# ZhonghuaYi/EI-Nexus_official

Hardware: AMD Instinct MI355X
Metric: event-image pairs/s (extract+match, 346x260, 1024 kpts) (higher is better)
Workload: dtype f32; 1 GPU; B32 346x260 5-bin event voxel + gray image, VGG(event)+SuperPoint(image) extractors, MNN matcher, k=1024; global_batch=32, event_bins=5, parallelism=dp1 (pairs sharded, metric all-reduce only), log_assignment=False, dense_outputs=False, same_scene_pairs=False, weights=seeded synthetic, descriptor-head bias calibrated (per-channel mean removed)

## Files before the change

### ei-nexus_official_amd/_lib.py

```python
import ctypes
import os

_HERE = os.path.dirname(os.path.abspath(__file__))
LIB_PATH = os.environ.get("EINX_LIB") or os.path.join(_HERE, "libeinx_hip.so")

c_void_p, c_int, c_float, c_size_t, c_char_p = ctypes.c_void_p, ctypes.c_int, ctypes.c_float, ctypes.c_size_t, ctypes.c_char_p


class ConvDesc(ctypes.Structure):
    _fields_ = [("w_native", c_void_p), ("bias", c_void_p), ("scale", c_void_p), ("shift", c_void_p),
                ("cin", ctypes.c_int32), ("cout", ctypes.c_int32), ("ks", ctypes.c_int32), ("relu", ctypes.c_int32),
                ("pool", ctypes.c_int32)]


class DetectParams(ctypes.Structure):
    _fields_ = [("B", ctypes.c_int32), ("Hp", ctypes.c_int32), ("Wp", ctypes.c_int32), ("H", ctypes.c_int32),
                ("W", ctypes.c_int32), ("h0", ctypes.c_int32), ("w0", ctypes.c_int32), ("radius", ctypes.c_int32),
                ("top_k", ctypes.c_int32), ("det_thr", c_float), ("ordering_xy", ctypes.c_int32), ("cap", ctypes.c_int32),
                ("nms_iters", ctypes.c_int32)]


class ExtractorDesc(ctypes.Structure):
    _fields_ = [("struct_size", c_size_t), ("cell", ctypes.c_int32), ("n_backbone", ctypes.c_int32), ("n_det", ctypes.c_int32), ("n_desc", ctypes.c_int32),
                ("backbone", ctypes.POINTER(ConvDesc)), ("det_head", ctypes.POINTER(ConvDesc)), ("desc_head", ctypes.POINTER(ConvDesc)),
# ... 11 lines not shown
              "sparse_desc")
    _fields_ = [(n, c_void_p) for n in _names] + [("cap", ctypes.c_int32), ("score_crop", c_void_p)]


class WeightWatch(ctypes.Structure):
    _fields_ = [("struct_size", c_size_t), ("n", ctypes.c_int32), ("table", c_void_p), ("ref", c_void_p), ("scratch", c_void_p), ("stale", c_void_p)]


class MetricParams(ctypes.Structure):
    _fields_ = [(n, ctypes.c_int32) for n in ("B", "cap0", "cap1", "D", "cols", "H0", "W0", "H1", "W1", "kp_yx", "n_mma", "n_vdd")] + \
               [("mma_thr", c_float * 4), ("vdd_thr", c_float * 4), ("rep_nan_if_empty", ctypes.c_int32)]


class PoseParams(ctypes.Structure):
    _fields_ = [("struct_size", c_size_t)] + [(n, ctypes.c_int32) for n in ("B", "cap", "cols", "kp_yx", "k_f64", "max_iters")] + \
               [("thresh", ctypes.c_double), ("conf", ctypes.c_double), ("seed", ctypes.c_uint64)]


class HomographyParams(ctypes.Structure):
    _fields_ = [("struct_size", c_size_t)] + [(n, ctypes.c_int32) for n in ("B", "cap", "cols", "kp_yx", "max_iters", "n_thr")] + \
               [("thresh", ctypes.c_double), ("conf", ctypes.c_double), ("he_thr", c_float * 4), ("seed", ctypes.c_uint64)]


class GtMatchesParams(ctypes.Structure):
    _fields_ = [("struct_size", c_size_t)] + [(n, ctypes.c_int32) for n in ("B", "cap0", "cap1", "cols0", "cols1", "kp_yx", "H0", "W0", "H1", "W1",
                                                                            "homography")] + [("pos_sq", c_float), ("neg_sq", c_float)]


class EventArrays(ctypes.Structure):
    _fields_ = [("x", c_void_p), ("y", c_void_p), ("t", c_void_p), ("p", c_void_p), ("x_type", ctypes.c_int32), ("y_type", ctypes.c_int32),
                ("t_type", ctypes.c_int32), ("p_type", ctypes.c_int32), ("n", ctypes.c_int64)]


class LgLayer(ctypes.Structure):
    _names = ("Wqkv", "bqkv", "Wo", "bo", "sf0_w", "sf0_b", "sln_g", "sln_b", "sf3_w", "sf3_b",
              "Wqk", "bqk", "Wv", "bv", "Wco", "bco", "cf0_w", "cf0_b", "cln_g", "cln_b", "cf3_w", "cf3_b", "Wqk_v", "bqk_v")
    _fields_ = [(n, c_void_p) for n in _names]


class LgWeights(ctypes.Structure):
    _fields_ = [("struct_size", c_size_t), ("layer_size", c_size_t), ("in_w", c_void_p), ("in_b", c_void_p), ("Wr", c_void_p), ("proj_w", c_void_p), ("proj_b", c_void_p),
                ("match_w", c_void_p), ("match_b", c_void_p), ("n_layers", ctypes.c_int32), ("heads", ctypes.c_int32),
                ("d", ctypes.c_int32), ("input_dim", ctypes.c_int32), ("filter_threshold", c_float),
                ("layers", ctypes.POINTER(LgLayer))]


class LgHead(ctypes.Structure):
    _fields_ = [(n, c_void_p) for n in ("proj_w", "proj_b", "match_w", "match_b", "token_w", "token_b")]


SIGNATURES = {
    "einx_version": (c_char_p, []),
    "einx_abi_version": (c_int, []),
    "einx_build_flags": (c_char_p, []),
    "einx_params_hash": (c_int, [c_void_p, c_int, c_void_p, c_void_p, c_void_p, c_void_p]),
    "einx_last_error": (c_char_p, []),
    "einx_math_eval": (c_int, [c_int, c_void_p, ctypes.c_longlong, c_void_p, c_void_p]),
    "einx_fork_stream_of": (c_void_p, [c_void_p]),
    "einx_fork_stream_prepare_beside": (c_int, [c_void_p, ctypes.POINTER(c_void_p), c_int]),
    "einx_stream_overlap_us": (c_int, [c_void_p, c_void_p, c_int, ctypes.POINTER(ctypes.c_float)]),
    "einx_device_count": (c_int, []),
    "einx_profile_enable": (c_int, [c_int]),
    "einx_profile_report": (c_int, [c_char_p, c_size_t]),
    "einx_extractor_create": (c_void_p, [ctypes.POINTER(ExtractorDesc)]),
    "einx_extractor_destroy": (None, [c_void_p]),
    "einx_fork_stream_prepare": (c_int, [c_void_p]),
    "einx_fork_stream_release": (c_int, [c_void_p]),
    "einx_fork_stream_count": (c_int, []),
    "einx_side_stream": (c_void_p, [c_void_p, c_int, ctypes.POINTER(c_void_p), c_int]),
    "einx_extract_shapes": (c_int, [c_void_p, c_int, c_int, ctypes.POINTER(ExtractShapes)]),
    "einx_extract_ws_bytes": (c_size_t, [c_void_p, c_int, c_int, c_int, c_int, c_int]),
    "einx_extract": (c_int, [c_void_p, c_void_p, c_void_p, c_int, c_int, c_int, c_int, c_void_p, c_size_t, ctypes.POINTER(ExtractOut), c_void_p]),
    "einx_extract_watch": (c_int, [c_void_p, c_void_p, c_void_p, c_int, c_int, c_int, c_int, c_void_p, c_size_t, ctypes.POINTER(ExtractOut),
                           ctypes.POINTER(WeightWatch), c_void_p]),
    "einx_conv_last_kernel": (c_char_p, []),
    "einx_conv_plan": (c_char_p, [c_int] * 11),
    "einx_conv_weight_elems": (c_size_t, [c_int, c_int, c_int]),
    "einx_conv_repack": (c_int, [c_void_p, c_int, c_int, c_int, c_void_p, c_void_p]),
    "einx_bn_fold": (c_int, [c_void_p, c_void_p, c_void_p, c_void_p, c_float, c_int, c_void_p, c_void_p, c_void_p]),
    "einx_conv_block": (c_int, [c_void_p, c_int, c_int, c_int, c_int, c_int, c_int, c_int, ctypes.POINTER(ConvDesc), c_void_p, c_void_p]),
    "einx_conv_first_two_fused_ok": (c_int, [ctypes.POINTER(ConvDesc), ctypes.POINTER(ConvDesc), c_int, c_int, c_int]),
    "einx_conv_first_two_fused": (c_int, [c_void_p, c_int, c_int, c_int, c_int, c_int, c_int, c_int, ctypes.POINTER(ConvDesc), ctypes.POINTER(ConvDesc),
                                  c_void_p, c_void_p]),
    "einx_div_inplace": (c_int, [c_void_p, c_size_t, c_float, c_void_p]),
    "einx_image_prepare": (c_int, [c_void_p, c_int, c_int, c_int, c_int, ctypes.c_longlong, ctypes.c_longlong, ctypes.c_longlong, ctypes.c_longlong,
                           c_float, c_void_p, c_void_p]),
    "einx_score_map": (c_int, [c_void_p, c_int, c_int, c_int, c_int, c_void_p, c_int, c_int, c_int, c_int, c_int, c_int, c_void_p,
                               c_void_p, c_void_p]),
    "einx_remove_border": (c_int, [c_void_p, c_int, c_int, c_int, c_int, c_void_p]),
    "einx_detect_ws_bytes": (c_size_t, [ctypes.POINTER(DetectParams)]),
    "einx_detect": (c_int, [c_void_p, ctypes.POINTER(DetectParams), c_void_p, c_void_p, c_void_p, c_void_p, c_void_p, c_void_p,
                            c_void_p, c_void_p]),
    "einx_desc_sample": (c_int, [c_void_p, c_int, c_int, c_int, c_int, c_int, c_int, c_int, c_int, c_void_p, c_void_p, c_int, c_float,
                                 c_void_p, c_void_p]),
    "einx_normalize_map": (c_int, [c_void_p, c_int, c_int, c_int, c_float, c_void_p, c_void_p, c_void_p]),
    "einx_upsample_ws_bytes": (c_size_t, [c_int, c_int, c_int]),
    "einx_upsample_normalize": (c_int, [c_void_p, c_int, c_int, c_int, c_int, c_int, c_int, c_int, c_int, c_int, c_int, c_float,
                                        c_void_p, c_void_p, c_size_t, c_void_p]),
    "einx_mnn_ws_bytes": (c_size_t, [c_int, c_int, c_int]),
    "einx_mnn": (c_int, [c_void_p, c_void_p, c_int, c_void_p, c_void_p, c_int, c_int, c_int, c_void_p, c_void_p, c_void_p, c_void_p,
                         c_void_p, c_void_p, c_void_p]),
    "einx_mnn_gather": (c_int, [c_void_p, c_void_p, c_int, c_void_p, c_void_p, c_int, c_int, c_int, c_void_p, c_void_p, c_void_p, c_void_p,
                                c_void_p, c_void_p, c_void_p, c_void_p, c_int, c_void_p, c_void_p, c_void_p, c_void_p]),
    "einx_mnn_thresh": (c_int, [c_void_p, c_void_p, c_int, c_void_p, c_void_p, c_int, c_int, c_int, c_int, c_float, c_int, c_float, c_void_p,
                                c_void_p, c_void_p, c_void_p, c_void_p, c_void_p, c_void_p]),
    "einx_gather_matches": (c_int, [c_void_p, c_void_p, c_void_p, c_void_p, c_int, c_int, c_int, c_int, c_void_p, c_void_p, c_void_p,
                                    c_void_p]),
    "einx_events_ws_bytes": (c_size_t, [c_int, c_int, c_int]),
    "einx_voxel_ws_bytes": (c_size_t, [c_int, c_int, c_int, c_int, ctypes.c_int64]),
    "einx_voxel_grid": (c_int, [c_void_p, c_void_p, c_void_p, c_void_p, c_void_p, c_int, c_int, c_int, c_int, c_int, c_void_p, c_void_p,
                                c_size_t, c_void_p]),
    "einx_events_mask": (c_int, [c_void_p, c_void_p, c_void_p, c_int, c_int, c_int, c_void_p, c_void_p, c_void_p]),
    "einx_time_surface_ws_bytes": (c_size_t, [c_int, c_int, c_int, c_int, ctypes.c_int64]),
    "einx_event_stack_ws_bytes": (c_size_t, [c_int, c_int, c_int, c_int, ctypes.c_int64]),
    "einx_distance_map_ws_bytes": (c_size_t, [c_int, c_int, c_int, c_int, ctypes.c_int64]),
    "einx_time_surface": (c_int, [c_void_p, c_void_p, c_void_p, c_void_p, c_void_p, c_int, c_int, c_int, c_int, c_void_p, c_void_p, c_size_t,
                                  c_void_p]),
    "einx_event_stack": (c_int, [c_void_p, c_void_p, c_void_p, c_void_p, c_void_p, c_int, c_int, c_int, c_int, c_void_p, c_void_p, c_size_t,
                                 c_void_p]),
    "einx_distance_map": (c_int, [c_void_p, c_void_p, c_void_p, c_void_p, c_void_p, c_int, c_int, c_int, c_int, c_void_p, c_void_p, c_size_t,
                                  c_void_p]),
    "einx_distance_map_plan": (c_char_p, [c_int, c_int]),
    "einx_events_windows_ws_bytes": (c_size_t, [c_int, c_int, c_int]),
    "einx_voxel_windows_ws_bytes": (c_size_t, [c_int, c_int, c_int, c_int, ctypes.c_int64]),
    "einx_voxel_grid_windows": (c_int, [c_void_p, c_void_p, c_void_p, c_void_p, ctypes.c_int64, c_void_p, c_void_p, c_int, c_int, c_int, c_int, c_int,
                                        c_void_p, c_void_p, c_size_t, c_void_p]),
    "einx_events_mask_windows": (c_int, [c_void_p, c_void_p, ctypes.c_int64, c_void_p, c_void_p, c_int, c_int, c_int, c_void_p, c_size_t, c_void_p,
                                         c_void_p]),
    "einx_events_pack": (c_int, [ctypes.POINTER(EventArrays), c_int, c_void_p, c_void_p, c_void_p, c_void_p, c_void_p, c_int]),
    "einx_metrics_ws_bytes": (c_size_t, [ctypes.POINTER(MetricParams)]),
    "einx_pair_metrics": (c_int, [ctypes.POINTER(MetricParams)] + [c_void_p] * 13),
    "einx_relative_pose_ws_bytes": (c_size_t, [ctypes.POINTER(PoseParams)]),
    "einx_relative_pose": (c_int, [ctypes.POINTER(PoseParams)] + [c_void_p] * 13),
    "einx_essential_5pt": (c_int, [c_void_p, c_void_p, c_int, c_void_p, c_void_p, c_void_p]),
    "einx_homography_ws_bytes": (c_size_t, [ctypes.POINTER(HomographyParams)]),
    "einx_homography": (c_int, [ctypes.POINTER(HomographyParams)] + [c_void_p] * 11),
    "einx_homography_dlt": (c_int, [c_void_p, c_void_p, c_int, c_int, c_void_p, c_void_p, c_void_p]),
    "einx_gt_matches_ws_bytes": (c_size_t, [ctypes.POINTER(GtMatchesParams)]),
    "einx_gt_project": (c_int, [ctypes.POINTER(GtMatchesParams)] + [c_void_p] * 23),
    "einx_gt_warp": (c_int, [ctypes.POINTER(GtMatchesParams)] + [c_void_p] * 8),
    "einx_gt_label": (c_int, [ctypes.POINTER(GtMatchesParams)] + [c_void_p] * 17),
    "einx_gt_matches": (c_int, [ctypes.POINTER(GtMatchesParams)] + [c_void_p] * 30),
    "einx_match_pr": (c_int, [c_void_p, c_void_p, c_void_p, c_void_p, c_int, c_int, c_void_p, c_void_p]),
    "einx_desc_loss_ws_bytes": (c_size_t, [c_int] * 11),
    "einx_desc_loss": (c_int, [c_void_p, c_float, c_void_p, c_float] + [c_int] * 11 + [c_void_p, c_int, c_int, c_void_p, c_void_p, c_size_t, c_void_p]),
    "einx_map_loss_ws_bytes": (c_size_t, [c_int, c_int]),
    "einx_map_loss": (c_int, [c_void_p, c_void_p, c_int, c_int, c_int, c_void_p, c_int, c_int, c_int, c_void_p, c_void_p, c_size_t, c_void_p]),
    "einx_logits_loss": (c_int, [c_void_p, c_void_p] + [c_int] * 9 + [c_void_p, c_int, c_void_p, c_void_p, c_size_t, c_void_p]),
    "einx_linear": (c_int, [c_void_p, c_int, c_int, c_void_p, c_void_p, c_int, c_void_p, c_int, c_void_p]),
    "einx_lg_ws_bytes": (c_size_t, [c_int, c_int, c_int, c_int, c_int]),
    "einx_lg_ws_bytes_heads": (c_size_t, [c_int, c_int, c_int, c_int, c_int, c_int]),
    "einx_lightglue": (c_int, [ctypes.POINTER(LgWeights), c_void_p, c_void_p, c_void_p, c_int, c_void_p, c_void_p, c_void_p, c_int,
                               c_int, c_float, c_float, c_float, c_float, c_void_p, c_void_p, c_void_p, c_void_p, c_void_p, c_void_p,
                               c_void_p, c_void_p, c_int, c_void_p]),
    "einx_lightglue_early_stop_ws_bytes": (c_size_t, [c_int] * 7),
    "einx_lightglue_early_stop": (c_int, [ctypes.POINTER(LgWeights), ctypes.POINTER(LgHead), c_size_t, c_float, c_void_p, c_void_p, c_void_p,
                                          c_int, c_void_p, c_void_p, c_void_p, c_int, c_int, c_float, c_float, c_float, c_float] + [c_void_p] * 10),
    "einx_lightglue_adaptive_ws_bytes": (c_size_t, [c_int] * 7),
    "einx_lightglue_adaptive": (c_int, [ctypes.POINTER(LgWeights), ctypes.POINTER(LgHead), c_size_t, c_float, ctypes.c_double, c_int, c_void_p,
                                        c_void_p, c_void_p, c_int, c_void_p, c_void_p, c_void_p, c_int, c_int, c_float, c_float, c_float, c_float]
                                + [c_void_p] * 15),
    "einx_lg_assign_nll_ws_bytes": (c_size_t, [c_int, c_int, c_int, c_int]),
    "einx_lg_assign_nll": (c_int, [c_void_p, c_void_p, c_void_p, c_void_p, c_int, c_void_p, c_void_p, c_int, c_void_p, c_void_p, c_int, c_int,
                                   c_void_p, c_void_p, c_void_p, c_void_p, ctypes.c_int64, ctypes.c_int64, ctypes.c_int64, c_void_p, c_void_p,
                                   c_void_p]),
    "einx_normalize_rows": (c_int, [c_void_p, c_int, c_int, c_float, c_void_p, c_void_p]),
# ... 41 lines not shown
```

### ei-nexus_official_amd/csrc/conv.hip

```cpp
#include <stdio.h>
#include <stdlib.h>

#include <type_traits>

#include "einx_common.h"

namespace {

constexpr int kCoutTile = 64;

struct ConvArgs {
  const float* in;
  const float* w;
  const float* bias;
  const float* scale;
  const float* shift;
  float* out;
  int B, Cin, Cout, CoutPad;
  int Hs, Ws, h0, w0;
  int H, W;
  int tilesX, tilesY;
  int relu;
};

// ... 789 lines not shown
  constexpr int CK = 32, G = CK / 4, NPX = 16 * NPW, WP = kCoutTile + 16;
  constexpr int IN_PER_THR = CK * NPX / 256, W_PER_THR = CK * (kCoutTile / 4) / 256;
  __shared__ __attribute__((aligned(16))) float in_tile[CK * NPX];
  __shared__ __attribute__((aligned(16))) float w_tile[CK * WP];
  const int tid = threadIdx.x, wave = tid >> 6, lane = tid & 63;
  const int q = lane >> 4, j = lane & 15;
  const int HW = a.H * a.W;
  const int tile = (int)blockIdx.x % a.tilesX, b = (int)blockIdx.x / a.tilesX;
  const int co0 = (int)blockIdx.y * kCoutTile;
  const int p0 = tile * NPX;
  const float* in_b = a.in + (size_t)b * a.Cin * HW;
  unsigned goff[IN_PER_THR], loff[IN_PER_THR];
#pragma unroll
  for (int i = 0; i < IN_PER_THR; ++i) {
    const int e = tid + i * 256;
    const int ch = e / NPX, px = e % NPX;
    goff[i] = (unsigned)ch * (unsigned)HW + (unsigned)min(p0 + px, HW - 1);
    loff[i] = (unsigned)e;
  }
  unsigned woff[W_PER_THR], wl[W_PER_THR];
#pragma unroll
  for (int i = 0; i < W_PER_THR; ++i) {
    const int f = tid + i * 256;
    const int r = f / (kCoutTile / 4), c4 = f % (kCoutTile / 4);
    woff[i] = (unsigned)(r * a.CoutPad + co0 + c4 * 4);
    wl[i] = (unsigned)(r * WP + c4 * 4);
  }
  float r_in[IN_PER_THR];
  f32x4 r_w[W_PER_THR];
  auto issue_loads = [&](int c) {
    const float* ib = in_b + (size_t)c * CK * HW;
#pragma unroll
    for (int i = 0; i < IN_PER_THR; ++i) r_in[i] = ib[goff[i]];
    const float* wb = a.w + (size_t)c * CK * a.CoutPad;
#pragma unroll
    for (int i = 0; i < W_PER_THR; ++i) r_w[i] = *reinterpret_cast<const f32x4*>(wb + woff[i]);
  };
  f32x4v acc[NPW];
#pragma unroll
  for (int n = 0; n < NPW; ++n) acc[n] = f32x4v{0.0f, 0.0f, 0.0f, 0.0f};
  const int nchunks = a.Cin / CK;
  issue_loads(0);
  float e_bi[4], e_sc[4], e_sh[4];
#pragma unroll
  for (int i = 0; i < 4; ++i) {
    const int coc = min(co0 + wave * 16 + 4 * q + i, a.Cout - 1);
    e_bi[i] = a.bias ? a.bias[coc] : 0.0f;
    e_sc[i] = a.scale ? a.scale[coc] : 1.0f;
    e_sh[i] = a.scale ? a.shift[coc] : 0.0f;
  }
  const int aoff = q * WP + wave * 16 + j, boff = q * NPX + j;
  for (int c = 0; c < nchunks; ++c) {
    __syncthreads();
#pragma unroll
    for (int i = 0; i < IN_PER_THR; ++i) in_tile[loff[i]] = r_in[i];
#pragma unroll
    for (int i = 0; i < W_PER_THR; ++i) *reinterpret_cast<f32x4*>(w_tile + wl[i]) = r_w[i];
    __syncthreads();
    if (c + 1 < nchunks) issue_loads(c + 1);
    float av[G], bv[G][NPW];
#pragma unroll
    for (int g = 0; g < G; ++g) {
      av[g] = w_tile[aoff + g * 4 * WP];
#pragma unroll
      for (int n = 0; n < NPW; ++n) bv[g][n] = in_tile[boff + g * 4 * NPX + 16 * n];
    }
#pragma unroll
    for (int g = 0; g < G; ++g)
#pragma unroll
      for (int n = 0; n < NPW; ++n) acc[n] = __builtin_amdgcn_mfma_f32_16x16x4f32(av[g], bv[g][n], acc[n], 0, 0, 0);
  }
  float* out_b = a.out + (size_t)b * a.Cout * HW;
#pragma unroll
  for (int i = 0; i < 4; ++i) {
    const int co = co0 + wave * 16 + 4 * q + i;
#pragma unroll
    for (int n = 0; n < NPW; ++n) {
      const int p = p0 + 16 * n + j;
      float v = acc[n][i] + e_bi[i];
      if (a.relu) v = v > 0.0f ? v : 0.0f;
      if (a.scale) v = fmaf(v, e_sc[i], e_sh[i]);
      if (co < a.Cout && p < HW) out_b[(size_t)co * HW + p] = v;
    }
  }
}

__global__ void conv_repack_kernel(const float* w, int cin, int cout, int taps, int coutPad, int krows, float* out) {
  const size_t n = (size_t)krows * coutPad;
  for (size_t i = (size_t)blockIdx.x * blockDim.x + threadIdx.x; i < n; i += (size_t)gridDim.x * blockDim.x) {
    const int co = (int)(i % coutPad);
    const int k = (int)(i / coutPad);
    const int h = k & 1;
    const int tap = (k >> 1) % taps;
    const int cp = (k >> 1) / taps;
    const int ci = 2 * cp + h;
    float v = 0.0f;
    if (ci < cin && co < cout) v = w[((size_t)co * cin + ci) * taps + tap];
    out[i] = v;
  }
}

__global__ void bn_fold_kernel(const float* g, const float* b, const float* mean, const float* var, float eps, int n, float* scale,
                               float* shift) {
  const int i = blockIdx.x * blockDim.x + threadIdx.x;
  if (i >= n) return;
  const float s = g[i] / sqrtf(var[i] + eps);
  scale[i] = s;
  shift[i] = b[i] - mean[i] * s;
}

int native_krows(int cin, int taps) { return einx_cdiv(cin, 32) * 32 * taps; }

thread_local const char* g_last_conv_kernel = "";

struct TileCfg {
  int th, tw, slots;
};

template <int KS, int TH, int TW, int WM, int WN, int MT, int NT, int CK, bool POOL, bool DENSE3 = false>
void launch(const ConvArgs& a, int B, hipStream_t s, bool three_per_cu = false) {
  dim3 grid((unsigned)(a.tilesX * a.tilesY * B), (unsigned)(a.CoutPad / kCoutTile));
  const bool three = DENSE3 && three_per_cu;
  {
    static char nm[2][96] = {{0}, {0}};
    char* n = nm[three ? 1 : 0];
    if (!n[0]) snprintf(n, sizeof nm[0], "conv_block_kernel<%d,%d,%d,%d,%d,%d,%d,%d,%s>%s", KS, TH, TW, WM, WN, MT, NT, CK, POOL ? "true" : "false", three ? " (3 per CU)" : "");
    g_last_conv_kernel = n;
  }
  EINX_PROF(KS == 1 ? "conv_block_kernel 1x1" : (CK < 8 ? "conv_block_kernel 3x3 first layer" : "conv_block_kernel 3x3"), s);
  if constexpr (DENSE3) {
    if (three) {
      hipLaunchKernelGGL((conv_block_kernel<KS, TH, TW, WM, WN, MT, NT, CK, POOL, false, 6>), grid, dim3(WM * WN * 64), 0, s, a);
      return;
    }
  }
  hipLaunchKernelGGL((conv_block_kernel<KS, TH, TW, WM, WN, MT, NT, CK, POOL>), grid, dim3(WM * WN * 64), 0, s, a);
}

double tile_waste(int H, int W, const TileCfg& c) {
  const double tiles = (double)einx_cdiv(H, c.th) * einx_cdiv(W, c.tw);
  return tiles * c.slots / ((double)H * W);
}

}

EINX_EXPORT const char* einx_conv_last_kernel(void) { return g_last_conv_kernel; }

EINX_EXPORT size_t einx_conv_weight_elems(int cin, int cout, int ks) {
  const int taps = ks * ks;
  const int coutPad = einx_cdiv(cout, kCoutTile) * kCoutTile;
  return (size_t)native_krows(cin, taps) * coutPad;
}

EINX_EXPORT int einx_conv_repack(const float* w_oihw, int cin, int cout, int ks, float* w_native, void* stream) {
  EINX_CHECK_ARG(w_oihw && w_native, "null pointer");
  EINX_CHECK_ARG(ks == 1 || ks == 3, "kernel size must be 1 or 3");
  EINX_CHECK_ARG(cin > 0 && cout > 0, "bad channel count");
  const int taps = ks * ks;
  const int coutPad = einx_cdiv(cout, kCoutTile) * kCoutTile;
  const int krows = native_krows(cin, taps);
  const size_t n = (size_t)krows * coutPad;
  const int blocks = (int)((n + 255) / 256 > 1024 ? 1024 : (n + 255) / 256);
  hipLaunchKernelGGL(conv_repack_kernel, dim3(blocks), dim3(256), 0, (hipStream_t)stream, w_oihw, cin, cout, taps, coutPad, krows,
                     w_native);
  EINX_CHECK_LAUNCH();
  return EINX_OK;
}

EINX_EXPORT int einx_bn_fold(const float* gamma, const float* beta, const float* mean, const float* var, float eps, int n, float* scale,
                             float* shift, void* stream) {
  EINX_CHECK_ARG(gamma && beta && mean && var && scale && shift, "null pointer");
  EINX_CHECK_ARG(n > 0, "bad channel count");
  hipLaunchKernelGGL(bn_fold_kernel, dim3(einx_cdiv(n, 256)), dim3(256), 0, (hipStream_t)stream, gamma, beta, mean, var, eps, n, scale,
                     shift);
  EINX_CHECK_LAUNCH();
  return EINX_OK;
}

EINX_EXPORT int einx_conv_first_two_fused_ok(const einx_conv_desc* d0, const einx_conv_desc* d1, int B, int H, int W) {
  if (!d0 || !d1) return 0;
  const bool shapes = (d0->cin == 1 || d0->cin == 5) && d0->cout == 64 && d0->ks == 3 && !d0->pool && d1->cin == 64 && d1->cout == 64 && d1->ks == 3;
  if (!shapes || (d1->pool && ((H & 1) || (W & 1)))) return 0;
  const long grid = (long)einx_cdiv(W, 32) * einx_cdiv(H, 8) * B;
  if (grid < 8L * 768) return 0;
  return d0->cin == 1 ? 1 : 2;
}

EINX_EXPORT int einx_conv_first_two_fused(const float* in, int B, int Hs, int Ws, int h0, int w0, int H, int W, const einx_conv_desc* d0,
                                          const einx_conv_desc* d1, float* out, void* stream) {
  EINX_CHECK_ARG(in && out && d0 && d1 && d0->w_native && d1->w_native, "null pointer");
  EINX_CHECK_ARG(einx_conv_first_two_fused_ok(d0, d1, B, H, W), "layers / launch size outside what the fused first-two-layers kernel covers");
  EINX_CHECK_ARG((d0->scale == nullptr) == (d0->shift == nullptr) && (d1->scale == nullptr) == (d1->shift == nullptr), "scale and shift go together");
  EINX_CHECK_ARG((size_t)d0->cin * Hs * Ws < (1u << 30) && (size_t)64 * H * W < (1u << 30), "image too large");
  Conv1abArgs fa;
  ConvArgs& a = fa.c;
  a.in = in;
  a.w = d1->w_native;
  a.bias = d1->bias;
  a.scale = d1->scale;
  a.shift = d1->shift;
  a.out = out;
  a.B = B;
  a.Cin = 64;
  a.Cout = 64;
  a.CoutPad = 64;
  a.Hs = Hs;
  a.Ws = Ws;
  a.h0 = h0;
  a.w0 = w0;
  a.H = H;
  a.W = W;
  a.relu = d1->relu;
  a.tilesX = einx_cdiv(W, 32);
  a.tilesY = einx_cdiv(H, 8);
  fa.w0 = d0->w_native;
  fa.bias0 = d0->bias;
  fa.scale0 = d0->scale;
  fa.shift0 = d0->shift;
  fa.relu0 = d0->relu;
  fa.cout0pad = 64;
  hipStream_t s = (hipStream_t)stream;
  dim3 grid((unsigned)(a.tilesX * a.tilesY * B), 1);
  static thread_local char nm[96];
  snprintf(nm, sizeof nm, "conv1ab_kernel<%d,%s> (first two layers fused, 3 per CU)", d0->cin, d1->pool ? "true" : "false");
  g_last_conv_kernel = nm;
  EINX_PROF("conv1ab_kernel (first two layers)", s);
  if (d0->cin == 1) {
    if (d1->pool) hipLaunchKernelGGL((conv1ab_kernel<1, true, 6>), grid, dim3(512), 0, s, fa);
    else hipLaunchKernelGGL((conv1ab_kernel<1, false, 6>), grid, dim3(512), 0, s, fa);
  } else {
    if (d1->pool) hipLaunchKernelGGL((conv1ab_kernel<5, true, 6>), grid, dim3(512), 0, s, fa);
    else hipLaunchKernelGGL((conv1ab_kernel<5, false, 6>), grid, dim3(512), 0, s, fa);
  }
  EINX_CHECK_LAUNCH();
  return EINX_OK;
}

namespace {

#define EINX_CONV_BLOCK_VARIANTS(X)                    \
  X(CB_1X1_128, 1, 1, 128, 1, 4, 2, 1, 32, false, false) \
  X(CB_1X1_256, 1, 1, 256, 1, 4, 2, 2, 32, false, false) \
  X(CB_P_8X32, 3, 8, 32, 2, 4, 1, 2, 8, true, true)      \
  X(CB_P_12X16, 3, 12, 16, 2, 2, 1, 3, 8, true, false)   \
  X(CB_P_22X8, 3, 22, 8, 2, 2, 1, 3, 8, true, false)     \
  X(CB_P_8X16, 3, 8, 16, 2, 2, 1, 2, 8, true, false)     \
  X(CB_P_4X16, 3, 4, 16, 2, 2, 1, 1, 8, true, false)     \
  X(CB_8X32_CK2, 3, 8, 32, 2, 4, 1, 2, 2, false, false)  \
  X(CB_8X32_CK6, 3, 8, 32, 2, 4, 1, 2, 6, false, false)  \
  X(CB_8X32, 3, 8, 32, 2, 4, 1, 2, 8, false, true)       \
  X(CB_12X16, 3, 12, 16, 2, 2, 1, 3, 8, false, false)    \
  X(CB_22X8, 3, 22, 8, 2, 2, 1, 3, 8, false, false)      \
  X(CB_11X22, 3, 11, 22, 2, 4, 1, 2, 8, false, false)    \
  X(CB_11X11, 3, 11, 11, 2, 2, 1, 2, 8, false, false)    \
  X(CB_11X5, 3, 11, 5, 2, 2, 1, 1, 8, false, false)

enum ConvVariant {
#define X(V, ...) V,
  EINX_CONV_BLOCK_VARIANTS(X)
#undef X
  CB_1X1_128_XTRA,
  C16_1X1,
  C16,
};

struct ConvPlan {
  int variant;
  int tilesX, tilesY;
  int npw;
  bool three;
};

struct ConvPlanLayer {
  int cin, cout, ks, pool;
};

void conv_plan_name(const ConvPlan& p, bool pool, char* nm, size_t n) {
  switch (p.variant) {
#define X(V, KS, TH, TW, WM, WN, MT, NT, CK, POOL, DENSE3)                                                                            \
  case V:                                                                                                                             \
    snprintf(nm, n, "conv_block_kernel<%d,%d,%d,%d,%d,%d,%d,%d,%s>%s", KS, TH, TW, WM, WN, MT, NT, CK, POOL ? "true" : "false", \
             DENSE3 && p.three ? " (3 per CU)" : "");                                                                                 \
    break;
    EINX_CONV_BLOCK_VARIANTS(X)
#undef X
    case CB_1X1_128_XTRA: snprintf(nm, n, "conv_block_kernel<1,1,128,1,4,2,1,32,false,xtra>"); break;
    case C16_1X1: snprintf(nm, n, "conv16_1x1_kernel<%d>", p.npw); break;
    default: snprintf(nm, n, "conv16_kernel<%s,8,%d>", pool ? "true" : "false", p.npw); break;
  }
}

const char* conv_shape_refused(const ConvPlanLayer* d, int B, int Hs, int Ws, int h0, int w0, int H, int W) {
  if (!(d->ks == 1 || d->ks == 3)) return "kernel size must be 1 or 3";
  if (!(B > 0 && H > 0 && W > 0 && Hs > 0 && Ws > 0 && d->cin > 0 && d->cout > 0)) return "bad shape";
  if (!(!d->pool || (H % 2 == 0 && W % 2 == 0))) return "pooling needs even H and W";
  if (!(d->ks == 3 || (Hs == H && Ws == W && h0 == 0 && w0 == 0))) return "1x1 layers take no padding fold";
  if (!(d->ks == 3 || !d->pool)) return "pooled 1x1 not supported";
  if (!((size_t)d->cin * Hs * Ws < (1u << 30) && (size_t)d->cout * H * W < (1u << 30) && (size_t)d->cin * H * W < (1u << 30)))
    return "image too large (2^30 elements per image and tensor)";
  return nullptr;
}

ConvPlan conv_plan(const ConvPlanLayer* d, int B, int Hs, int Ws, int h0, int w0, int H, int W) {
  ConvPlan p = {0, 0, 0, 0, false};
  const int CoutPad = einx_cdiv(d->cout, kCoutTile) * kCoutTile;
  if (d->ks == 1) {
    const long blocks256 = (long)einx_cdiv(H * W, 256) * B * (CoutPad / kCoutTile);
    p.tilesY = 1;
    {
      const long max_wg128 = 512;
      const long blocks128 = (long)einx_cdiv(H * W, 128) * B * (CoutPad / kCoutTile);
      if (blocks128 < max_wg128 && d->cin % 32 == 0) {
        int npw = 1;
        for (int cand = 4; cand > 1; cand >>= 1)
          if ((long)einx_cdiv(H * W, 16 * cand) * B * (CoutPad / kCoutTile) >= 512) {
            npw = cand;
            break;
          }
        p.tilesX = einx_cdiv(H * W, 16 * npw);
        p.variant = C16_1X1;
        p.npw = npw;
// ... 205 lines not shown
```

### ei-nexus_official_amd/csrc/extract.hip

```cpp
#include <stdlib.h>
#include <string.h>

#include <algorithm>
#include <mutex>
#include <new>
#include <vector>

#include "einx_common.h"

struct einx_extractor {
  einx_extractor_desc d;
  std::vector<einx_conv_desc> backbone, det, desc;
  bool has_merged = false;
  einx_conv_desc merged;
};

namespace {

struct Plan {
  int Hp, Wp, h0, w0;
  int hc, wc;
  size_t buf_elems[2];
  size_t head_elems;
};
// ... 140 lines not shown
  return EINX_OK;
}

static inline int nms_budget(int nms_iters) { return nms_iters > 0 ? nms_iters : 8; }

namespace {
struct ExtractWs {
  float* buf[2];
  float *head, *head2;
  void* det_ws;
  EinxDetectWs det;
};

ExtractWs carve(WsCarver& c, const einx_extractor* e, const Plan& pl, const einx_detect_params* dp, int B) {
  ExtractWs w;
  w.buf[0] = c.take<float>(pl.buf_elems[0] * B);
  w.buf[1] = c.take<float>(pl.buf_elems[1] * B);
  w.head = c.take<float>(pl.head_elems * B);
  w.head2 = fork_heads(e, pl, B) ? c.take<float>(pl.head_elems * B) : w.head;
  w.det_ws = c.here();
  w.det = einx_detect_carve(c, dp);
  c.slack(256);
  return w;
}
}

EINX_EXPORT size_t einx_extract_ws_bytes(const einx_extractor* e, int B, int H, int W, int cap, int nms_iters) {
  Plan pl;
  if (!e || B <= 0 || !make_plan(e, H, W, &pl)) return 0;
  einx_detect_params p;
  detect_params(e, pl, B, H, W, cap > 0 ? cap : 1, nms_budget(nms_iters), &p);
  WsCarver c{nullptr};
  carve(c, e, pl, &p, B);
  return c.bytes;
}

EINX_EXPORT int einx_extract(const einx_extractor* e, float* in, const uint8_t* mask, int B, int H, int W, int nms_iters, void* ws,
                             size_t ws_bytes, const einx_extract_out* o, void* stream) {
  return einx_extract_watch(e, in, mask, B, H, W, nms_iters, ws, ws_bytes, o, nullptr, stream);
}

EINX_EXPORT int einx_extract_watch(const einx_extractor* e, float* in, const uint8_t* mask, int B, int H, int W, int nms_iters, void* ws,
                                   size_t ws_bytes, const einx_extract_out* o, const einx_weight_watch* ww, void* stream) {
  EINX_CHECK_ARG(e && in && ws && o, "null pointer");
  EINX_CHECK_ARG(!ww || ww->struct_size == sizeof(einx_weight_watch), "einx_weight_watch::struct_size does not match this library (ABI mismatch)");
  EINX_CHECK_ARG(!ww || ww->n == 0 || (ww->n > 0 && ww->table && ww->ref && ww->scratch && ww->stale), "weight watch with null pointers");
  EINX_CHECK_ARG(o->feats && o->logits && o->raw && o->prob && o->score && o->positions && o->indices && o->counts && o->thr &&
                     o->not_converged && o->sparse_desc,
                 "null output pointer");
  EINX_CHECK_ARG(B > 0 && H > 0 && W > 0 && o->cap > 0, "bad shape");
  Plan pl;
  EINX_CHECK_ARG(make_plan(e, H, W, &pl), "image size does not fit the network's pooling / cell size");
  EINX_CHECK_ARG(e->d.cell == 1 || (o->coarse && o->raw_cl), "cell-8 networks need the coarse / raw_cl outputs");
  EINX_CHECK_ARG(ws_bytes >= einx_extract_ws_bytes(e, B, H, W, o->cap, nms_iters), "workspace smaller than einx_extract_ws_bytes for these arguments");
  einx_detect_params dp;
  detect_params(e, pl, B, H, W, o->cap, nms_budget(nms_iters), &dp);
  WsCarver c{(char*)ws};
  const ExtractWs wk = carve(c, e, pl, &dp, B);
  bool fork = fork_heads(e, pl, B) && !einx_profile_active();
  {
    hipStreamCaptureStatus cs = hipStreamCaptureStatusNone;
    if (fork && hipStreamIsCapturing((hipStream_t)stream, &cs) == hipSuccess && cs != hipStreamCaptureStatusNone) fork = false;
  }
  float* const head2 = fork ? wk.head2 : wk.head;
  int rc;
  if (e->d.input_div != 0.0f && e->d.input_div != 1.0f) {
    rc = einx_div_inplace(in, (size_t)B * e->backbone.front().cin * H * W, e->d.input_div, stream);
    if (rc) return rc;
  }
  const float* cur = in;
  int h = pl.Hp, w = pl.Wp;
  const int nb = (int)e->backbone.size();
  int first = 0;
  if (nb >= 2 && 1 == einx_conv_first_two_fused_ok(&e->backbone[0], &e->backbone[1], B, pl.Hp, pl.Wp)) {
    float* out = (2 < nb) ? wk.buf[1] : o->feats;
    if ((rc = einx_conv_first_two_fused(in, B, H, W, pl.h0, pl.w0, pl.Hp, pl.Wp, &e->backbone[0], &e->backbone[1], out, stream))) return rc;
    if (e->backbone[1].pool) {
      h /= 2;
      w /= 2;
    }
    cur = out;
    first = 2;
  }
  for (int i = first; i < nb; ++i) {
    const einx_conv_desc& c = e->backbone[i];
    float* out = (i + 1 < nb) ? wk.buf[i & 1] : o->feats;
    if (i == 0) rc = einx_conv_block(cur, B, H, W, pl.h0, pl.w0, pl.Hp, pl.Wp, &c, out, stream);
    else rc = einx_conv_block(cur, B, h, w, 0, 0, h, w, &c, out, stream);
    if (rc) return rc;
    if (c.pool) {
      h /= 2;
      w /= 2;
    }
    cur = out;
  }
  auto run_head = [&](const std::vector<einx_conv_desc>& L, float* scratch, float* final_out, void* st) -> int {
    const float* x = o->feats;
    for (size_t i = 0; i < L.size(); ++i) {
      float* out = (i + 1 < L.size()) ? scratch : final_out;
      const int r = einx_conv_block(x, B, h, w, 0, 0, h, w, &L[i], out, st);
      if (r) return r;
      x = out;
    }
    return 0;
  };
  const int D = e->desc.back().cout;
  const bool merged = e->has_merged && B == 1;
  if (merged && (rc = einx_conv_block(o->feats, B, h, w, 0, 0, h, w, &e->merged, wk.head, stream))) return rc;
  const float* desc_in = wk.head + (size_t)e->det.front().cout * h * w;
  auto det_branch = [&](void* st) -> int {
    if (merged) return einx_conv_block(wk.head, B, h, w, 0, 0, h, w, &e->det[1], o->logits, st);
    return run_head(e->det, wk.head, o->logits, st);
  };
  auto desc_branch = [&](void* st) -> int {
    int r = merged ? einx_conv_block(desc_in, B, h, w, 0, 0, h, w, &e->desc[1], o->raw, st) : run_head(e->desc, head2, o->raw, st);
    if (r) return r;
    if (e->d.cell == 8) r = einx_normalize_map(o->raw, B, D, h * w, e->d.desc_scale, o->coarse, o->raw_cl, st);
    return r;
  };
  std::unique_lock<std::mutex> side_lock;
  const EinxSide* sd = fork ? einx_side_acquire((hipStream_t)stream, &side_lock) : nullptr;
  if (sd) {
    if (hipEventRecord(sd->fork, (hipStream_t)stream) != hipSuccess || hipStreamWaitEvent(sd->stream, sd->fork, 0) != hipSuccess) {
      einx_set_error("einx_extract: fork failed");
      return EINX_ERR_LAUNCH;
    }
    rc = desc_branch(sd->stream);
    const bool ok = hipEventRecord(sd->join, sd->stream) == hipSuccess;
    if (rc) {
      (void)hipStreamWaitEvent((hipStream_t)stream, sd->join, 0);
      return rc;
    }
    if (!ok) {
      einx_set_error("einx_extract: join failed");
      return EINX_ERR_LAUNCH;
    }
    if ((rc = det_branch(stream))) {
      (void)hipStreamWaitEvent((hipStream_t)stream, sd->join, 0);
      return rc;
    }
  } else {
    if ((rc = det_branch(stream))) return rc;
    if ((rc = desc_branch(stream))) return rc;
  }
  const int C_det = e->det.back().cout;
  const long score_threads = (long)(C_det == 65 ? einx_cdiv(B * h * w, 32) : einx_cdiv(B * h * w, 256)) * 256;
  const bool zero_in_score = wk.det.nflags > 0 && wk.det.nflags <= score_threads;
  rc = einx_score_map_zero(o->logits, B, C_det, h, w, mask, H, W, pl.h0, pl.w0, e->d.dilate_mask, e->d.border, o->prob, o->score,
                           zero_in_score ? wk.det.flags : nullptr, zero_in_score ? wk.det.nflags : 0, o->score_crop, stream);
  if (rc) {
    if (sd) (void)hipStreamWaitEvent((hipStream_t)stream, sd->join, 0);
    return rc;
  }
  const float* nms_map = nullptr;
  rc = einx_detect_prezeroed(o->score, &dp, wk.det_ws, o->nms, o->positions, o->indices, o->counts, o->thr, o->not_converged, zero_in_score ? 1 : 0,
                             o->nms ? &nms_map : nullptr, stream);
  if (sd && hipStreamWaitEvent((hipStream_t)stream, sd->join, 0) != hipSuccess && !rc) {
    einx_set_error("einx_extract: join failed");
    return EINX_ERR_LAUNCH;
  }
  if (rc) return rc;
  const bool bilinear = e->d.cell == 8;
  const bool use_cl = bilinear && D <= 512;
  EinxWatch watch;
  const bool on = ww && ww->n > 0;
  watch.table = on ? ww->table : nullptr;
  watch.ref = on ? (const unsigned long long*)ww->ref : nullptr;
  watch.hash = on ? (unsigned long long*)ww->scratch : nullptr;
  watch.flag = on ? ww->stale : nullptr;
  watch.n = on ? ww->n : 0;
  watch.bit = 1;
  EinxCrop crop{};
  crop.map = o->nms ? nms_map : nullptr;
  crop.thr = o->thr;
  crop.out = o->nms;
  crop.Hp = pl.Hp;
  crop.Wp = pl.Wp;
  crop.h0 = pl.h0;
  crop.w0 = pl.w0;
  crop.H = H;
  crop.W = W;
  return einx_desc_sample_watch(use_cl ? o->raw_cl : o->raw, B, D, h, w, pl.Hp, pl.Wp, bilinear ? 1 : 0, use_cl ? 1 : 0, o->indices, o->counts,
                                o->cap, e->d.desc_scale, o->sparse_desc, watch, crop, stream);
// ... 2 lines not shown
```

### include/einx.h

```cpp
#ifndef EINX_H
#define EINX_H

#include <stddef.h>
#include <stdint.h>

#ifdef __cplusplus
extern "C" {
#endif

#define EINX_OK 0
#define EINX_ERR_ARG (-1)
#define EINX_ERR_LAUNCH (-2)
#define EINX_ERR_NO_DEVICE (-3)

#define EINX_ABI_VERSION 6
int einx_abi_version(void);
const char* einx_version(void);
const char* einx_last_error(void);
const char* einx_build_flags(void);
int einx_device_count(void);

#define EINX_WATCH_CHUNK_WORDS 4096
int einx_params_hash(const int64_t* table, int n, uint64_t* hash, const uint64_t* ref, int32_t* stale, void* stream);

int einx_math_eval(int fn, const float* x, long long n, float* y, void* stream);

int einx_stream_overlap_us(void* stream_a, void* stream_b, int spin_us, float* elapsed_us);

int einx_profile_enable(int on);
int einx_profile_report(char* buf, size_t cap);


size_t einx_conv_weight_elems(int cin, int cout, int ks);
int einx_conv_repack(const float* w_oihw, int cin, int cout, int ks, float* w_native, void* stream);

int einx_bn_fold(const float* gamma, const float* beta, const float* mean, const float* var, float eps, int n, float* scale,
                 float* shift, void* stream);

typedef struct einx_conv_desc {
  const float* w_native;
  const float* bias;
  const float* scale;
  const float* shift;
  int32_t cin, cout, ks;
  int32_t relu;
  int32_t pool;
} einx_conv_desc;

int einx_conv_block(const float* in, int B, int Hs, int Ws, int h0, int w0, int H, int W, const einx_conv_desc* d, float* out,
                    void* stream);

int einx_conv_first_two_fused_ok(const einx_conv_desc* d0, const einx_conv_desc* d1, int B, int H, int W);
int einx_conv_first_two_fused(const float* in, int B, int Hs, int Ws, int h0, int w0, int H, int W, const einx_conv_desc* d0,
                              const einx_conv_desc* d1, float* out, void* stream);

const char* einx_conv_last_kernel(void);

const char* einx_conv_plan(int cin, int cout, int ks, int pool, int B, int Hs, int Ws, int h0, int w0, int H, int W);

int einx_div_inplace(float* x, size_t n, float divisor, void* stream);

int einx_image_prepare(float* image, int B, int C, int H, int W, long long stride_b, long long stride_c, long long stride_h,
                       long long stride_w, float divisor, float* gray, void* stream);


int einx_score_map(const float* logits, int B, int C, int hc, int wc, const uint8_t* mask, int H, int W, int h0, int w0,
                   int dilate, int border, float* prob, float* score, void* stream);

int einx_remove_border(float* score, int B, int Hp, int Wp, int border, void* stream);

int einx_dense_positions(const float* score, int B, int H, int W, int ordering_xy, float* out, void* stream);

typedef struct einx_detect_params {
  int32_t B, Hp, Wp;
  int32_t H, W, h0, w0;
  int32_t radius;
  int32_t top_k;
  float det_thr;
  int32_t ordering_xy;
  int32_t cap;
  int32_t nms_iters;
} einx_detect_params;

size_t einx_detect_ws_bytes(const einx_detect_params* p);

int einx_detect(const float* score, const einx_detect_params* p, void* ws, float* nms_out, float* positions, int32_t* indices,
                int32_t* counts, float* thr, int32_t* not_converged, void* stream);


int einx_desc_sample(const float* raw, int B, int D, int hc, int wc, int Hp, int Wp, int bilinear, int channels_last,
                     const int32_t* indices, const int32_t* counts, int cap, float scale, float* out, void* stream);

int einx_normalize_map(const float* raw, int B, int D, int P, float scale, float* out, float* raw_cl, void* stream);

int einx_normalize_rows(const float* x, int R, int C, float scale, float* out, void* stream);

int einx_random_positions(const float* u, int R, float size0, float size1, float* out, void* stream);

size_t einx_upsample_ws_bytes(int B, int H, int W);
int einx_upsample_normalize(const float* raw, int B, int D, int hc, int wc, int Hp, int Wp, int h0, int w0, int H, int W,
                            float scale, float* out, void* ws, size_t ws_bytes, void* stream);

size_t einx_mnn_ws_bytes(int B, int cap0, int cap1);
int einx_mnn(const float* desc0, const int32_t* n, int cap0, const float* desc1, const int32_t* m, int cap1, int B, int D,
             void* ws, int64_t* matches0, int64_t* matches1, float* scores0, float* scores1, float* la, void* stream);
int einx_mnn_gather(const float* desc0, const int32_t* n, int cap0, const float* desc1, const int32_t* m, int cap1, int B, int D,
                    void* ws, int64_t* matches0, int64_t* matches1, float* scores0, float* scores1, float* la, const float* kpts0,
                    const float* kpts1, int cols, float* mk0, float* mk1, int32_t* nmatch, void* stream);
int einx_mnn_thresh(const float* desc0, const int32_t* n, int cap0, const float* desc1, const int32_t* m, int cap1, int B, int D,
                    int use_ratio, float ratio_sq, int use_dist, float dist_sq, void* ws, int64_t* matches0, int64_t* matches1,
                    float* scores0, float* scores1, float* la, void* stream);

int einx_similarity(const float* desc0, const int32_t* n, int cap0, const float* desc1, const int32_t* m, int cap1, int B, int D,
                    float* sim, void* stream);

int einx_gather_matches(const float* kpts0, const float* kpts1, const int64_t* matches0, const int32_t* n, int cap0, int cap1,
                        int B, int cols, float* out0, float* out1, int32_t* nmatch, void* stream);

int einx_compact_rows(const float* src0, const float* src1, const int32_t* counts, int B, int cap, int width, float* dst0, float* dst1,
                      void* stream);

int einx_linear(const float* x, int M, int K, const float* w, const float* bias, int N, float* y, int accumulate, void* stream);

typedef struct einx_lg_layer {
  const float *Wqkv, *bqkv, *Wo, *bo, *sf0_w, *sf0_b, *sln_g, *sln_b, *sf3_w, *sf3_b;
  const float *Wqk, *bqk, *Wv, *bv, *Wco, *bco, *cf0_w, *cf0_b, *cln_g, *cln_b, *cf3_w, *cf3_b;
  const float *Wqk_v, *bqk_v;
} einx_lg_layer;

typedef struct einx_lg_weights {
  size_t struct_size;
  size_t layer_size;
  const float* in_w;
  const float* in_b;
  const float* Wr;
  const float* proj_w;
  const float* proj_b;
// ... 240 lines not shown
```

Measured before the change: 3852 pairs/s.

## Add full-width strip 3x3 conv kernel for 88-wide feature maps

Adds a specialized 3x3 MFMA convolution kernel where each workgroup covers a two-row strip spanning the full 88-pixel width for one 64-channel output tile. Input chunks are prefetched to registers and committed to a bank-conflict-padded LDS tile while MFMAs run on the previous chunk; pooling is fused in the epilogue via lane shuffles. It is selected for backbone and head layers when the map width is exactly 88 and enough workgroups exist, with an environment override. It aims to cut halo redundancy and improve data reuse over the generic tiled conv, at the cost of a shape-specific code path.

After: 3811 pairs/s. 1.1% lower.

```diff
diff --git a/ei-nexus_official_amd/_lib.py b/ei-nexus_official_amd/_lib.py
--- a/ei-nexus_official_amd/_lib.py
+++ b/ei-nexus_official_amd/_lib.py
@@ -117,6 +117,8 @@
     "einx_conv_first_two_fused_ok": (c_int, [ctypes.POINTER(ConvDesc), ctypes.POINTER(ConvDesc), c_int, c_int, c_int]),
     "einx_conv_first_two_fused": (c_int, [c_void_p, c_int, c_int, c_int, c_int, c_int, c_int, c_int, ctypes.POINTER(ConvDesc), ctypes.POINTER(ConvDesc),
                                   c_void_p, c_void_p]),
+    "einx_conv_strip16_ok": (c_int, [ctypes.POINTER(ConvDesc), c_int, c_int, c_int]),
+    "einx_conv_strip16": (c_int, [c_void_p, c_int, c_int, c_int, ctypes.POINTER(ConvDesc), c_void_p, c_void_p]),
     "einx_div_inplace": (c_int, [c_void_p, c_size_t, c_float, c_void_p]),
     "einx_image_prepare": (c_int, [c_void_p, c_int, c_int, c_int, c_int, ctypes.c_longlong, ctypes.c_longlong, ctypes.c_longlong, ctypes.c_longlong,
                            c_float, c_void_p, c_void_p]),
diff --git a/ei-nexus_official_amd/csrc/conv.hip b/ei-nexus_official_amd/csrc/conv.hip
--- a/ei-nexus_official_amd/csrc/conv.hip
+++ b/ei-nexus_official_amd/csrc/conv.hip
@@ -895,6 +895,178 @@
       if (a.scale) v = fmaf(v, e_sc[i], e_sh[i]);
       if (co < a.Cout && p < HW) out_b[(size_t)co * HW + p] = v;
     }
+  }
+}
+
+template <bool POOL>
+__global__ __launch_bounds__(256, 4) void conv_strip16_kernel(const ConvArgs a) {
+  constexpr int NPW = 11, CK = 8, TAPS = 9, KCH = CK * TAPS, G = KCH / 4;
+  constexpr int TW = 8 * NPW, PH = 4, PW = TW + 2;
+  constexpr int PITCH = 104, PLANE = PH * PITCH + 16;
+  static_assert(PITCH >= PW && PITCH % 32 == 8 && PLANE % 32 == 16, "rows 8 banks apart, channel parities 16");
+  constexpr int PLANE_E = PH * PW;
+  constexpr int CPT = 4, NGRP = CK / CPT;
+  constexpr int ITEMS = PLANE_E * NGRP;
+  constexpr int IPT = (ITEMS + 255) / 256;
+  constexpr int W_F4 = KCH * kCoutTile / 4;
+  constexpr int W_PER_THR = (W_F4 + 255) / 256;
+  static_assert(W_F4 % 64 == 0, "the weight tail is whole waves");
+  __shared__ __attribute__((aligned(16))) float in_tile[CK * PLANE];
+  __shared__ __attribute__((aligned(16))) float w_tile[KCH * kCoutTile];
+  __shared__ __attribute__((aligned(16))) float s_bias[kCoutTile], s_scale[kCoutTile], s_shift[kCoutTile];
+  const int tid = threadIdx.x;
+  const int wave = __builtin_amdgcn_readfirstlane(tid >> 6);
+  const int lane = tid & 63;
+  const int q = lane >> 4, j = lane & 15;
+  const int ncot = (int)gridDim.y;
+  const int item = xcd_contiguous((int)(blockIdx.x + blockIdx.y * gridDim.x), (int)gridDim.x * ncot);
+  const int co0 = (item % ncot) * kCoutTile;
+  const int bid = item / ncot;
+  const int y0 = (bid % a.tilesY) * 2;
+  const int b = bid / a.tilesY;
+  if (tid < kCoutTile) {
+    const int co = co0 + tid;
+    const bool cv = co < a.Cout;
+    s_bias[tid] = (cv && a.bias) ? a.bias[co] : 0.0f;
+    s_scale[tid] = (cv && a.scale) ? a.scale[co] : 1.0f;
+    s_shift[tid] = (cv && a.scale) ? a.shift[co] : 0.0f;
+  }
+  const unsigned HW = (unsigned)(a.H * a.W);
+  const float* in_b = a.in + (size_t)b * a.Cin * HW;
+  unsigned in_voff[IPT];
+  int lds_pos[IPT];
+  unsigned okmask = 0;
+#pragma unroll
+  for (int i = 0; i < IPT; ++i) {
+    const int e = tid + i * 256;
+    const bool live = e < ITEMS;
+    const int pos = e % PLANE_E, grp = live ? e / PLANE_E : 0;
+    const int py = pos / PW, px = pos % PW;
+    const int y = y0 - 1 + py, x = px - 1;
+    const bool inside = live && y >= 0 && y < a.H && x >= 0 && x < a.W;
+    in_voff[i] = ((unsigned)(inside ? y * a.W + x : 0) + (unsigned)(grp * CPT) * HW) * 4u;
+    lds_pos[i] = grp * CPT * PLANE + py * PITCH + px;
+    okmask |= (inside ? 1u : 0u) << i;
+    if (live && !inside) {
+#pragma unroll
+      for (int ch = 0; ch < CPT; ++ch) in_tile[lds_pos[i] + ch * PLANE] = 0.0f;
+    }
+  }
+  const unsigned woff = (unsigned)((tid >> 4) * a.CoutPad + co0 + (tid & 15) * 4) * 4u;
+  const int bpix = (j >> 3) * PITCH + (j & 7) + (q & 1) * PLANE;
+  const int b_col = bpix + (q >> 1);
+  const int b_row = bpix + (q >> 1) * (PITCH - 2);
+  const int b_pair = bpix + (q >> 1) * (2 * PLANE - 2 * PITCH - 2);
+  const int aoff = q * kCoutTile + wave * 16 + j;
+  struct StageRegs {
+    float in[IPT][CPT];
+    f32x4 w[W_PER_THR];
+  };
+  StageRegs sA;
+  auto issue_loads = [&](int c) {
+    const int ci0 = c * CK;
+    __amdgpu_buffer_rsrc_t rs[CPT];
+#pragma unroll
+    for (int ch = 0; ch < CPT; ++ch) rs[ch] = conv_rsrc(in_b + (size_t)(ci0 + ch) * HW, (unsigned)(a.Cin - ci0 - ch) * HW * 4u);
+#pragma unroll
+    for (int i = 0; i < IPT; ++i)
+      if ((okmask >> i) & 1u) {
+#pragma unroll
+        for (int ch = 0; ch < CPT; ++ch) sA.in[i][ch] = __builtin_bit_cast(float, __builtin_amdgcn_raw_buffer_load_b32(rs[ch], in_voff[i], 0, 0));
+      }
+#pragma unroll
+    for (int i = 0; i < W_PER_THR; ++i)
+      if ((i + 1) * 256 <= W_F4 || tid + i * 256 < W_F4) {
+        const int rows = (i + 1) * 256 <= W_F4 ? 16 : (W_F4 - i * 256) / 16;
+        const __amdgpu_buffer_rsrc_t rw = conv_rsrc(a.w + (size_t)(c * KCH + 16 * i) * a.CoutPad, (unsigned)(rows * a.CoutPad) * 4u);
+        sA.w[i] = __builtin_bit_cast(f32x4, __builtin_amdgcn_raw_buffer_load_b128(rw, woff, 0, 0));
+      }
+  };
+  auto commit_loads = [&]() {
+#pragma unroll
+    for (int i = 0; i < IPT; ++i)
+      if ((okmask >> i) & 1u) {
+#pragma unroll
+        for (int ch = 0; ch < CPT; ++ch) in_tile[lds_pos[i] + ch * PLANE] = sA.in[i][ch];
+      }
+#pragma unroll
+    for (int i = 0; i < W_PER_THR; ++i)
+      if ((i + 1) * 256 <= W_F4 || tid + i * 256 < W_F4) *reinterpret_cast<f32x4*>(w_tile + (tid + i * 256) * 4) = sA.w[i];
+  };
+  f32x4v acc[NPW];
+#pragma unroll
+  for (int n = 0; n < NPW; ++n) acc[n] = f32x4v{0.0f, 0.0f, 0.0f, 0.0f};
+  auto mfma_chunk = [&]() {
+    float av[2], bv[2][NPW];
+    auto load_frag = [&](int g, int buf) {
+      const int k0 = 4 * g, pair = k0 / (2 * TAPS), tap = (k0 % (2 * TAPS)) >> 1;
+      const int base = tap == TAPS - 1 ? b_pair : (tap % 3 == 2 ? b_row : b_col);
+      const int koff = 2 * pair * PLANE + (tap / 3) * PITCH + tap % 3;
+      av[buf] = w_tile[aoff + g * 4 * kCoutTile];
+#pragma unroll
+      for (int n = 0; n < NPW; ++n) bv[buf][n] = in_tile[base + koff + 8 * n];
+    };
+    load_frag(0, 0);
+#pragma unroll
+    for (int g = 0; g < G; ++g) {
+      if (g + 1 < G) load_frag(g + 1, (g + 1) & 1);
+      __builtin_amdgcn_sched_barrier(0);
+#pragma unroll
+      for (int n = 0; n < NPW; ++n) acc[n] = __builtin_amdgcn_mfma_f32_16x16x4f32(av[g & 1], bv[g & 1][n], acc[n], 0, 0, 0);
+      __builtin_amdgcn_sched_barrier(0);
+    }
+  };
+  const int nchunks = a.Cin / CK;
+  issue_loads(0);
+  for (int c = 0; c < nchunks; ++c) {
+    __syncthreads();
+    commit_loads();
+    __syncthreads();
+    if (c + 1 < nchunks) issue_loads(c + 1);
+    mfma_chunk();
+  }
+  const int ty = j >> 3, tx = j & 7;
+  const int Ho = POOL ? a.H / 2 : a.H, Wo = POOL ? a.W / 2 : a.W;
+  const unsigned plane_o = (unsigned)(Ho * Wo);
+  float* out_b = a.out + (size_t)b * a.Cout * plane_o;
+  const bool st = POOL ? (ty == 0 && !(tx & 1)) : (y0 + ty < a.H);
+  const unsigned ov = POOL ? ((unsigned)((y0 >> 1) * Wo + (tx >> 1)) + (unsigned)(4 * q) * plane_o) * 4u
+                           : ((unsigned)((y0 + ty) * a.W + tx) + (unsigned)(4 * q) * plane_o) * 4u;
+  constexpr unsigned NSTEP = POOL ? 16u : 32u;
+  const int cw0 = co0 + wave * 16;
+  auto epilogue = [&](auto relu_c, auto aff_c) {
+    constexpr bool RELU = decltype(relu_c)::value, AFF = decltype(aff_c)::value;
+    const f32x4 bi = *reinterpret_cast<const f32x4*>(&s_bias[wave * 16 + 4 * q]);
+    f32x4 sc, sh;
+    if (AFF) {
+      sc = *reinterpret_cast<const f32x4*>(&s_scale[wave * 16 + 4 * q]);
+      sh = *reinterpret_cast<const f32x4*>(&s_shift[wave * 16 + 4 * q]);
+    }
+#pragma unroll
+    for (int i = 0; i < 4; ++i) {
+      const int nch = a.Cout - (cw0 + i) > 0 ? a.Cout - (cw0 + i) : 0;
+      const __amdgpu_buffer_rsrc_t ro = conv_rsrc(out_b + (size_t)(cw0 + i) * plane_o, (unsigned)nch * plane_o * 4u);
+#pragma unroll
+      for (int n = 0; n < NPW; ++n) {
+        float v = acc[n][i] + bi[i];
+        if (RELU) v = fmaxf(v, 0.0f);
+        if (AFF) v = fmaf(v, sc[i], sh[i]);
+        if (POOL) {
+          v = max_lane_xor<8>(v);
+          v = max_lane_xor<1>(v);
+        }
+        if (st) __builtin_amdgcn_raw_buffer_store_b32(__builtin_bit_cast(unsigned, v), ro, ov + n * NSTEP, 0, 0);
+      }
+    }
+  };
+  using T_ = std::integral_constant<bool, true>;
+  using F_ = std::integral_constant<bool, false>;
+  if (a.relu) {
+    if (a.scale) epilogue(T_{}, T_{});
+    else epilogue(T_{}, F_{});
+  } else {
+    if (a.scale) epilogue(F_{}, T_{});
+    else epilogue(F_{}, F_{});
   }
 }
 
@@ -1050,6 +1222,57 @@
 }
 
 namespace {
+bool strip16_covers(const einx_conv_desc* d, int B, int H, int W) {
+  if (!d || d->ks != 3 || d->cin <= 0 || d->cin % 8 != 0 || d->cout <= 0) return false;
+  if (B <= 0 || H <= 0 || W != 88 || (d->pool && (H & 1))) return false;
+  return (size_t)d->cin * H * W < (1u << 30) && ((size_t)d->cout + 16) * H * W < (1u << 30);
+}
+constexpr long kStrip16MinWorkgroupsPooled = 512, kStrip16MinWorkgroupsPlain = 4096;
+}
+
+EINX_EXPORT int einx_conv_strip16_ok(const einx_conv_desc* d, int B, int H, int W) {
+  if (!strip16_covers(d, B, H, W)) return 0;
+  const char* sw = getenv("EINX_STRIP16");
+  if (sw && (sw[0] == '0' || sw[0] == '1') && !sw[1]) return sw[0] == '1' ? 1 : 2;
+  const int CoutPad = einx_cdiv(d->cout, kCoutTile) * kCoutTile;
+  return (long)einx_cdiv(H, 2) * B * (CoutPad / kCoutTile) >= (d->pool ? kStrip16MinWorkgroupsPooled : kStrip16MinWorkgroupsPlain) ? 1 : 2;
+}
+
+EINX_EXPORT int einx_conv_strip16(const float* in, int B, int H, int W, const einx_conv_desc* d, float* out, void* stream) {
+  EINX_CHECK_ARG(in && out && d && d->w_native, "null pointer");
+  EINX_CHECK_ARG((d->scale == nullptr) == (d->shift == nullptr), "scale and shift go together");
+  EINX_CHECK_ARG(strip16_covers(d, B, H, W), "layer / map outside what the strip kernel covers (3x3, cin % 8 == 0, W == 88, even H when pooled)");
+  ConvArgs a;
+  a.in = in;
+  a.w = d->w_native;
+  a.bias = d->bias;
+  a.scale = d->scale;
+  a.shift = d->shift;
+  a.out = out;
+  a.B = B;
+  a.Cin = d->cin;
+  a.Cout = d->cout;
+  a.CoutPad = einx_cdiv(d->cout, kCoutTile) * kCoutTile;
+  a.Hs = H;
+  a.Ws = W;
+  a.h0 = 0;
+  a.w0 = 0;
+  a.H = H;
+  a.W = W;
+  a.relu = d->relu;
+  a.tilesX = 1;
+  a.tilesY = einx_cdiv(H, 2);
+  hipStream_t s = (hipStream_t)stream;
+  dim3 grid((unsigned)(a.tilesY * B), (unsigned)(a.CoutPad / kCoutTile));
+  g_last_conv_kernel = d->pool ? "conv_strip16_kernel<true>" : "conv_strip16_kernel<false>";
+  EINX_PROF("conv_block_kernel 3x3 strip16", s);
+  if (d->pool) hipLaunchKernelGGL(conv_strip16_kernel<true>, grid, dim3(256), 0, s, a);
+  else hipLaunchKernelGGL(conv_strip16_kernel<false>, grid, dim3(256), 0, s, a);
+  EINX_CHECK_LAUNCH();
+  return EINX_OK;
+}
+
+namespace {
 
 #define EINX_CONV_BLOCK_VARIANTS(X)                    \
   X(CB_1X1_128, 1, 1, 128, 1, 4, 2, 1, 32, false, false) \
diff --git a/ei-nexus_official_amd/csrc/extract.hip b/ei-nexus_official_amd/csrc/extract.hip
--- a/ei-nexus_official_amd/csrc/extract.hip
+++ b/ei-nexus_official_amd/csrc/extract.hip
@@ -246,11 +246,15 @@
     cur = out;
     first = 2;
   }
+  auto conv_layer = [&](const float* x, const einx_conv_desc& c, float* out, void* st) -> int {
+    if (einx_conv_strip16_ok(&c, B, h, w) == 1) return einx_conv_strip16(x, B, h, w, &c, out, st);
+    return einx_conv_block(x, B, h, w, 0, 0, h, w, &c, out, st);
+  };
   for (int i = first; i < nb; ++i) {
     const einx_conv_desc& c = e->backbone[i];
     float* out = (i + 1 < nb) ? wk.buf[i & 1] : o->feats;
     if (i == 0) rc = einx_conv_block(cur, B, H, W, pl.h0, pl.w0, pl.Hp, pl.Wp, &c, out, stream);
-    else rc = einx_conv_block(cur, B, h, w, 0, 0, h, w, &c, out, stream);
+    else rc = conv_layer(cur, c, out, stream);
     if (rc) return rc;
     if (c.pool) {
       h /= 2;
@@ -262,7 +266,7 @@
     const float* x = o->feats;
     for (size_t i = 0; i < L.size(); ++i) {
       float* out = (i + 1 < L.size()) ? scratch : final_out;
-      const int r = einx_conv_block(x, B, h, w, 0, 0, h, w, &L[i], out, st);
+      const int r = conv_layer(x, L[i], out, st);
       if (r) return r;
       x = out;
     }
diff --git a/include/einx.h b/include/einx.h
--- a/include/einx.h
+++ b/include/einx.h
@@ -53,6 +53,9 @@
 int einx_conv_first_two_fused_ok(const einx_conv_desc* d0, const einx_conv_desc* d1, int B, int H, int W);
 int einx_conv_first_two_fused(const float* in, int B, int Hs, int Ws, int h0, int w0, int H, int W, const einx_conv_desc* d0,
                               const einx_conv_desc* d1, float* out, void* stream);
+
+int einx_conv_strip16_ok(const einx_conv_desc* d, int B, int H, int W);
+int einx_conv_strip16(const float* in, int B, int H, int W, const einx_conv_desc* d, float* out, void* stream);
 
 const char* einx_conv_last_kernel(void);
 
```
